# raviraj988/3D-POINT-CLOUD-SEGMENTATION-USING-2D-IMG-SEGMENTATION

Measured on AMD Instinct MI355X. Metric: labelled points/sec (10M pts x 64 views) at 1/2/4/8 GPU; % HBM roofline, higher is better.
Workload: dtype f64; 1 GPU; C3: 10000000 points x 64 ring views, 1024x1024 block64 uint8 masks, nclasses=133, threshold=0.5, filter_classes=None; fused project->sample->vote->segment; points_total=10000000, points_per_gpu=10000000, views=64, xyz_storage=f64, cloud_layout=caller order, cell-sorted inside every step (F3D_FUSE_SORT), exchange=none

## Files before the change

3d-point-cloud-segmentation-using-2d-img-segmentation_amd/csrc/f3d_fuse.hip:

```cpp
#include <hip/hip_runtime.h>
#include <stdint.h>
#include <stdlib.h>
#include <string.h>
#include "f3d.h"
#include "f3d_math.h"
#include "f3d_kernels.h"
#include "f3d_fuse_blocks.h"
#include "f3d_fuse_deal.h"
#include <cstdlib>

#pragma clang fp contract(off)

#define F3D_NO_PREFILL ((int64_t)0x7fffffffffffffffLL)
#define F3D_PART_MAX_GROUPS 16
#ifndef F3D_MID_DENSE
#define F3D_MID_DENSE 8
#endif
#ifndef F3D_NT_CLASSES
#define F3D_NT_CLASSES 1
#endif
#if defined(F3D_EXP_STORE) && F3D_EXP_STORE == 2
#define F3D_STORE_CLASS(p, v) ((void)(v))
#elif defined(F3D_EXP_STORE) && F3D_EXP_STORE == 3
#define F3D_STORE_CLASS(p, v) (reinterpret_cast<uint8_t*>(classes)[(p) - classes] = (uint8_t)(v))
// ... 1357 lines not shown
        if (nclasses + 3 > F3D_BIN32_MAX_CODES) fuse(km2, lds_mid, F3D_BIN32_MAX_CODES + 1, 4 * F3D_PACKED_SMALL_WORDS, one_group ? 4 : 3);
        if (nclasses + 3 > 4 * F3D_PACKED_SMALL_WORDS) fuse(km3, lds_large, 4 * F3D_PACKED_SMALL_WORDS + 1, 4 * F3D_PACKED_LARGE_WORDS, 3);
        if (nclasses + 3 > 4 * F3D_PACKED_LARGE_WORDS) fuse(kf, lds_full, 4 * F3D_PACKED_LARGE_WORDS + 1, 256, 2);
        if (chunk_flags & 2) return hipGetLastError();
        const bool wide = nviews > 255;
        if (wide && !j.masks) return hipErrorInvalidValue;
        auto km = k_fuse_mid<T, V>;
        const size_t lds_tier2 = mid_lds_bytes(words_max);
        if ((e = raise_lds(km, lds_tier2)) != hipSuccess) return e;
        hipLaunchKernelGGL(km, dim3(1024), b, lds_tier2, s, xyz, todo_count, todo, j.views_dev, nviews, j.cmasks, h, w, nclasses, flt.nfilter,
                           flt.cls_dev, j.threshold, j.classes, j.votes, j.err, j.perm, gather, wide ? todo_count + 2 : (unsigned int*)nullptr,
                           wide ? todo2 : (int32_t*)nullptr, todo2_count, j.cb,
                           (const unsigned long long*)umask, (const uint32_t*)park, j.lay.park_slots, j.lay.park_stride);
        if (!wide) return hipGetLastError();
    }
    const unsigned int* exact_count = fast ? todo_count + 2 : todo2_count;
    const int32_t* exact_list = fast ? todo2 : nullptr;
    auto ke = mode == MODE_HIST8 ? k_fuse_exact<T, MODE_HIST8, V> : k_fuse_exact<T, MODE_HIST16, V>;
    if ((e = raise_lds(ke, lds_exact)) != hipSuccess) return e;
    hipLaunchKernelGGL(ke, ge, b, lds_exact, s, xyz, n, exact_count, exact_list, j.views_dev, nviews, j.masks, h, w, nclasses,
                       flt, j.threshold, j.classes, j.votes, j.err, j.perm, gather);
    return hipGetLastError();
}

static f3d_setup_args setup_args_for(const f3d_fuse_job& j, f3d_codebook* cb, bool with_book) {
    const int v0 = j.carry ? j.v0 : 0, cnv = (j.carry ? j.v1 : j.nviews) - v0;
    const fuse_tables tab = fuse_tables_split(j.tables, cnv);
    f3d_setup_args a;
    a.views = j.views_dev + v0; a.nviews = cnv; a.ctabT = tab.ctabT; a.vtabT = tab.vtabT; a.cb = cb; a.threshold = j.threshold;
    a.todo_count = v0 == 0 ? f3d_fuse_todo::counters(j.todo) : (unsigned int*)nullptr;
    a.lut_nclasses = with_book ? j.nclasses : 0;
    a.lut_book = with_book ? pick_book(j.flt, j.votes != nullptr) : -1;
    a.flt = j.flt;
    if (!with_book) { a.flt.nfilter = 0; a.flt.cls_dev = nullptr; a.flt.cls_host = nullptr; for (int k = 0; k < 8; ++k) a.flt.cls[k] = -1; }
    return a;
}

hipError_t f3d_launch_fuse_setup(const f3d_fuse_job& j, f3d_codebook* cb, bool with_book) {
    if ((j.carry ? j.v1 - j.v0 : j.nviews) <= 0) return hipSuccess;
    if (with_book && (j.nclasses < 0 || j.nclasses > F3D_CODE_MAX_NCLASSES)) return hipErrorInvalidValue;
    hipLaunchKernelGGL(k_fuse_setup, dim3(with_book ? 9 : 8), dim3(F3D_BLOCK), 0, j.stream, setup_args_for(j, cb, with_book));
    return hipGetLastError();
}

hipError_t f3d_launch_cell_sort_with_riders(f3d_fuse_job& j, uint8_t* coded, f3d_codebook* cb, int32_t* perm, void* sort_scratch) {
    if (j.nviews <= 0 || j.n <= 0) return hipErrorInvalidValue;
    if (j.nclasses < 0 || j.nclasses > F3D_CODE_MAX_NCLASSES || ((uintptr_t)coded & 7)) return hipErrorInvalidValue;
    f3d_sort_riders r;
    r.masks = j.masks; r.mask_bytes = (int64_t)j.nviews * j.h * j.w; r.cb = cb;
    r.presence = pick_book(j.flt, j.votes != nullptr) == 1;
    const int64_t fill = unlabelled_after_remap(j.nclasses, j.flt);
    j.filled = fill != F3D_NO_PREFILL;
    r.classes = j.filled ? j.classes : nullptr; r.n = j.n; r.fill_value = fill;
    const int pb = r.presence ? f3d_grid_for(r.mask_bytes >> 4, F3D_RIDER_THREADS * F3D_RIDER_UNROLL_1, F3D_RIDER_BLOCKS_1) : 0;
    const int fb = j.filled ? f3d_grid_for(j.n, F3D_RIDER_THREADS * 8, F3D_RIDER_BLOCKS_1) : 0;
    r.pass1_blocks = pb > fb ? pb : fb;
    r.setup = setup_args_for(j, cb, true); r.setup_blocks = 9;
    r.coded = coded; r.V = j.nviews; r.H = j.h; r.W = j.w;
    r.code_blocks = f3d_grid_for((int64_t)j.nviews * (int64_t)(f3d_coded_plane(j.h, j.w) / 8), F3D_RIDER_THREADS * F3D_RIDER_UNROLL, F3D_RIDER_BLOCKS_2);
    return f3d_launch_cell_sort(j.xyz, j.dtype, j.n, nullptr, perm, sort_scratch, j.stream, &r);
}

hipError_t f3d_launch_fuse(const f3d_fuse_job& j) {
    if (j.n <= 0) return hipSuccess;
    const int mode = j.nviews <= 255 ? MODE_HIST8 : MODE_HIST16;
    const int64_t ntiles = (j.n + F3D_BLOCK * 2 - 1) / (F3D_BLOCK * 2);
    int grid = (int)(ntiles < F3D_FUSE_GRID ? ntiles : F3D_FUSE_GRID);
    grid = (grid + 7) & ~7;
    if (j.carry && j.votes) return hipErrorInvalidValue;
    if (j.carry) return j.dtype == F3D_F64 ? launch_fuse_t<double, false, true>(j, mode, grid) : launch_fuse_t<float, false, true>(j, mode, grid);
    if (j.dtype == F3D_F64) return j.votes ? launch_fuse_t<double, true, false>(j, mode, grid) : launch_fuse_t<double, false, false>(j, mode, grid);
    return j.votes ? launch_fuse_t<float, true, false>(j, mode, grid) : launch_fuse_t<float, false, false>(j, mode, grid);
}

hipError_t f3d_launch_fastpath_audit(const void* xyz, int dtype, int64_t n, const f3d_view* views_dev, int nviews, int w, int h,
                                     unsigned long long* stats_dev, hipStream_t s) {
    hipError_t e = hipMemsetAsync(stats_dev, 0, 4 * sizeof(unsigned long long), s);
    if (e != hipSuccess || n <= 0) return e;
    const dim3 g(f3d_grid_for(n, F3D_BLOCK, F3D_GRID_CAP)), b(F3D_BLOCK);
    if (dtype == F3D_F64) hipLaunchKernelGGL(k_fastpath_audit<double>, g, b, 0, s, (const double*)xyz, n, views_dev, nviews, w, h, stats_dev);
    else hipLaunchKernelGGL(k_fastpath_audit<float>, g, b, 0, s, (const float*)xyz, n, views_dev, nviews, w, h, stats_dev);
    return hipGetLastError();
}
```

3d-point-cloud-segmentation-using-2d-img-segmentation_amd/csrc/f3d_fuse_blocks.h:

```cpp
#pragma once
#include <hip/hip_runtime.h>
#include <stdint.h>
#include "f3d.h"
#include "f3d_kernels.h"

#define F3D_RIDER_THREADS 512
#ifndef F3D_RIDER_UNROLL
#define F3D_RIDER_UNROLL 6
#endif
#ifndef F3D_RIDER_UNROLL_1
#define F3D_RIDER_UNROLL_1 8
#endif
#ifndef F3D_RIDER_BLOCKS_1
#define F3D_RIDER_BLOCKS_1 256
#endif
#ifndef F3D_RIDER_BLOCKS_2
#define F3D_RIDER_BLOCKS_2 1024
#endif
#define F3D_CODE_NONE 0u
#define F3D_CODE_BAD 1u
#define F3D_CODE_OTHER 2u
#define F3D_VHEAD 15

__host__ __device__ inline int f3d_coded_pitch(int W) { return ((W + 7) >> 3) + 2; }
__host__ __device__ inline size_t f3d_coded_plane(int H, int W) { return (size_t)(((H + 7) >> 3) + 2) * (size_t)f3d_coded_pitch(W) * 64; }

__device__ __forceinline__ void f3d_presence_publish(const unsigned* blkset, f3d_codebook* __restrict__ cb) {
    if (threadIdx.x < 8) {
        const unsigned want = blkset[threadIdx.x];
        const unsigned have = __hip_atomic_load(&cb->presence[threadIdx.x], __ATOMIC_RELAXED, __HIP_MEMORY_SCOPE_AGENT);
        if (want & ~have) atomicOr(&cb->presence[threadIdx.x], want);
    }
}

template <bool VEC>
__device__ __forceinline__ void f3d_presence_block(const uint8_t* __restrict__ src, int64_t nbytes, f3d_codebook* __restrict__ cb,
                                                   int blk, int nblk, int nthr) {
    unsigned long long m0 = 0, m1 = 0, m2 = 0, m3 = 0;
    auto mark = [&](unsigned l) {
        const unsigned long long bit = 1ull << (l & 63u);
        const unsigned q = l >> 6;
        m0 |= q == 0u ? bit : 0ull; m1 |= q == 1u ? bit : 0ull; m2 |= q == 2u ? bit : 0ull; m3 |= q == 3u ? bit : 0ull;
    };
    const int64_t stride = (int64_t)nblk * nthr;
    if (VEC) {
        const int64_t nw = nbytes >> 3;
        const uint64_t* w = reinterpret_cast<const uint64_t*>(src);
        uint64_t last = ~0ull;
        for (int64_t k = (int64_t)blk * nthr + threadIdx.x; k < nw; k += stride) {
            const uint64_t x = w[k];
            if (x == last) continue;
            if (x == (x & 0xFFull) * 0x0101010101010101ull) { mark((unsigned)(x & 0xFFull)); last = x; continue; }
#pragma unroll
            for (int c = 0; c < 8; ++c) mark((unsigned)(x >> (8 * c)) & 0xFFu);
        }
        if (blk == 0 && (int64_t)threadIdx.x < (nbytes & 7)) mark(src[(nw << 3) + threadIdx.x]);
    } else {
        for (int64_t k = (int64_t)blk * nthr + threadIdx.x; k < nbytes; k += stride) mark(src[k]);
    }
#pragma unroll
    for (int off = 32; off >= 1; off >>= 1) {
        m0 |= __shfl_xor(m0, off, 64); m1 |= __shfl_xor(m1, off, 64); m2 |= __shfl_xor(m2, off, 64); m3 |= __shfl_xor(m3, off, 64);
    }
    __shared__ unsigned blkset[8];
    if (threadIdx.x < 8) blkset[threadIdx.x] = 0u;
    __syncthreads();
    if ((threadIdx.x & 63) == 0) {
        const unsigned long long m[4] = {m0, m1, m2, m3};
#pragma unroll
        for (int q = 0; q < 4; ++q) {
// ... 167 lines not shown
                xs[u] = in[u] ? *reinterpret_cast<const uint64_t*>(rows + ry * W + tx * 8) : 0ull;
            }
#pragma unroll
            for (int u = 0; u < UNROLL; ++u) {
                const int e = e0 + 64 * u;
                if (e >= per_row) break;
                const uint64_t x = xs[u];
                uint64_t o = 0;
                if (in[u]) {
                    if (x == ((x << 8) | (x >> 56))) { const uint32_t c = (uint32_t)lut[x & 0xFFull] * 0x01010101u; o = ((uint64_t)c << 32) | c; }
                    else {
#pragma unroll
                        for (int c = 0; c < 8; ++c) o |= (uint64_t)lut[(x >> (8 * c)) & 0xFFull] << (8 * c);
                    }
                }
                out[e] = o;
            }
        }
    }
}

__device__ __forceinline__ void f3d_fill_labels_block(int64_t* __restrict__ classes, int64_t n, int64_t value, int blk, int nblk, int nthr) {
    for (int64_t i = (int64_t)blk * nthr + threadIdx.x; i < n; i += (int64_t)nblk * nthr)
        __builtin_nontemporal_store(value, &classes[i]);
}

struct f3d_setup_args {
    const f3d_view* views; int nviews;
    float* ctabT; double* vtabT;
    f3d_codebook* cb; double threshold;
    unsigned int* todo_count;
    int lut_nclasses, lut_book;
    f3d_filter_args flt;
};
__device__ __forceinline__ void f3d_fuse_setup_block(const f3d_setup_args& a, int blk, int nblk, int nthr) {
    if (a.lut_book >= 0 && blk == nblk - 1) { f3d_code_lut_block(a.cb, a.lut_nclasses, a.lut_book, a.flt); return; }
    if (blk == 0) {
        f3d_threshold_table(a.cb, a.threshold);
        if (a.todo_count && threadIdx.x < 4) a.todo_count[threadIdx.x] = 0u;
    }
    const int ngroups = (a.nviews + 63) >> 6;
    const int nsetup = a.lut_book >= 0 ? nblk - 1 : nblk;
    for (int k = blk * nthr + threadIdx.x; k < ngroups * 64 * 39; k += nsetup * nthr) {
        const int v = k / 39, f = k - v * 39, g = v >> 6, l = v & 63;
        const f3d_view& vw = a.views[v < a.nviews ? v : a.nviews - 1];
        if (f < 24) a.ctabT[(g * 24 + f) * 64 + l] = reinterpret_cast<const float*>(&vw.cull_n32[0][0])[f];
        else a.vtabT[(g * F3D_VHEAD + (f - 24)) * 64 + l] = reinterpret_cast<const double*>(&vw)[f - 24];
    }
}

struct f3d_sort_riders {
    const uint8_t* masks; int64_t mask_bytes; f3d_codebook* cb; bool presence;
    int64_t* classes; int64_t n; int64_t fill_value; int pass1_blocks;
    f3d_setup_args setup; int setup_blocks;
    uint8_t* coded; int V, H, W; int code_blocks;
};
```

3d-point-cloud-segmentation-using-2d-img-segmentation_amd/csrc/f3d_kernels.h:

```cpp
#pragma once
#include <hip/hip_runtime.h>
#include <float.h>
#include <stdint.h>
#include <atomic>
#include "f3d.h"
#include "f3d_math.h"

#define F3D_DEVERR_FUSE 1
#define F3D_DEVERR_VOTE 2
#define F3D_DEVERR_CC 4
#define F3D_DEVERR_FLOOD 8
#define F3D_DEVERR_COLOR 16
#define F3D_DEVERR_QUADS 32
#define F3D_DEVERR_GROW 64
#define F3D_DEVERR_PVOTE 128
#define F3D_DEVERR_MESH 256
#define F3D_DEVERR_ZVOTE 512
#define F3D_DEVERR_PLANES 1024
#define F3D_DEVERR_RASTER 2048
#define F3D_DEVERR_SMOOTH 4096
#define F3D_DEVERR_LIFT 8192
#define F3D_DEVERR_ALL 16383
#define F3D_PLANES_PER_LAUNCH 16
#define F3D_OBB_MAX_BOXES 4096
// ... 266 lines not shown
hipError_t f3d_launch_inside_polyhedra(const void* xyz, int dtype, int64_t n, const f3d_plane_args& pa, uint8_t* inside,
                                       hipStream_t s);
#define F3D_CODE_MAX_NCLASSES 253
struct f3d_fuse_todo {
    size_t bytes, list2_off, umask_off, park_off;
    int park_slots, park_stride, ngroups;
    static unsigned int* counters(void* base) { return reinterpret_cast<unsigned int*>(base); }
    static int32_t* list(void* base) { return reinterpret_cast<int32_t*>(reinterpret_cast<char*>(base) + 4 * sizeof(unsigned int)); }
    int32_t* list2(void* base) const { return reinterpret_cast<int32_t*>(reinterpret_cast<char*>(base) + list2_off); }
    unsigned long long* umask(void* base) const { return reinterpret_cast<unsigned long long*>(reinterpret_cast<char*>(base) + umask_off); }
    uint32_t* park(void* base) const { return reinterpret_cast<uint32_t*>(reinterpret_cast<char*>(base) + park_off); }
};
f3d_fuse_todo f3d_fuse_todo_layout(int64_t n, int nviews, int nclasses);
size_t f3d_fuse_tables_bytes(int nviews);
size_t f3d_fuse_carry_bytes(int64_t n, int nclasses);
struct f3d_fuse_occupancy {
    struct entry { const void* kernel; size_t lds; int blocks_per_cu; } e[32];
    int n, cus;
};
struct f3d_fuse_job {
    const void* xyz; int dtype; int64_t n; const int32_t* perm; bool gather;
    const f3d_view* views_dev; int nviews, v0, v1;
    const uint8_t *masks, *cmasks; int h, w;
    int nclasses; f3d_filter_args flt; double threshold;
    int64_t* classes; uint16_t* votes; int* err;
    void* todo; f3d_fuse_todo lay;
    const f3d_codebook* cb; void* tables; uint32_t* carry; void* xyz_keep;
    hipStream_t stream;
    bool filled;
    f3d_fuse_occupancy* occ;
};
hipError_t f3d_launch_fuse(const f3d_fuse_job& job);
hipError_t f3d_launch_fuse_setup(const f3d_fuse_job& job, f3d_codebook* cb, bool with_book);
hipError_t f3d_launch_code_masks_with_setup(const f3d_fuse_job& job, uint8_t* coded, f3d_codebook* cb);
hipError_t f3d_launch_mask_presence(const uint8_t* src, int64_t nbytes, f3d_codebook* cb, hipStream_t s);
hipError_t f3d_launch_presence_bytes(f3d_codebook* cb, uint8_t* bytes256, bool to_bytes, hipStream_t s);
hipError_t f3d_launch_code_book(f3d_codebook* cb, int nclasses, const f3d_filter_args& flt, bool want_votes, hipStream_t s);
hipError_t f3d_launch_code_planes(const uint8_t* src, uint8_t* dst, int nviews, int h, int w, const f3d_codebook* cb, hipStream_t s);
size_t f3d_coded_masks_bytes(int nviews, int h, int w);
hipError_t f3d_launch_fastpath_audit(const void* xyz, int dtype, int64_t n, const f3d_view* views_dev, int nviews, int w, int h,
                                     unsigned long long* stats_dev, hipStream_t s);
size_t f3d_sort_scratch_bytes(int64_t n);
struct f3d_sort_riders;
hipError_t f3d_launch_cell_sort(const void* xyz, int dtype, int64_t n, void* sorted_xyz, int32_t* perm, void* scratch, hipStream_t s,
                                const f3d_sort_riders* riders = nullptr);
struct f3d_block_role { bool rider; int index; };
__host__ __device__ inline f3d_block_role f3d_rider_role(unsigned b, unsigned grid, unsigned extra) {
    const unsigned before = (unsigned)(((unsigned long long)b * extra) / grid);
    const unsigned upto = (unsigned)(((unsigned long long)(b + 1) * extra) / grid);
    f3d_block_role r;
    r.rider = upto != before;
    r.index = r.rider ? (int)before : (int)(b - before);
    return r;
}
hipError_t f3d_launch_cell_sort_with_riders(f3d_fuse_job& job, uint8_t* coded, f3d_codebook* cb, int32_t* perm, void* sort_scratch);
hipError_t f3d_launch_components(const int64_t* classes, int64_t n, const int64_t* offs, const int32_t* nbrs, int32_t* parent,
                                 int64_t* root, int* err, hipStream_t s, int errbit = F3D_DEVERR_CC);
size_t f3d_flood_scratch_bytes(int64_t n);
hipError_t f3d_launch_flood_order(const int64_t* classes, int64_t n, const int64_t* offs, const int32_t* nbrs, const int64_t* inst, int k,
                                  int64_t* root, int64_t* order, int64_t* coffs, uint8_t* flags, void* scratch, int* err, int64_t stats[4],
                                  hipStream_t s);
struct f3d_color_args {
    double thr[3];
    int max_level;
    int nneutral;
    int64_t neutral[F3D_COLOR_MAX_NEUTRAL];
};
size_t f3d_color_scratch_bytes(int64_t n);
hipError_t f3d_launch_color_segment(const void* colors, int dtype, int64_t n, const int64_t* offs, const int32_t* nbrs, int64_t* ids,
                                    const int64_t* seeds, int64_t nseeds, const f3d_color_args& a, void* scratch, int64_t* stats_dev, int* err,
                                    hipStream_t s);
struct f3d_grow_args {
    double thr[3];
    double sma0[3];
    int64_t npts0;
    int max_level;
    int seeds_given;
};
#define F3D_GROW_MAX_POINTS (0x7fffffffLL - 2048)
size_t f3d_grow_scratch_bytes(int64_t n);
hipError_t f3d_launch_region_grow(const void* values, int dtype, int nchan, int64_t n, const int64_t* offs, const int32_t* nbrs,
                                  const int64_t* seeds, int64_t nseeds, const f3d_grow_args& a, void* scratch, int64_t* cluster,
                                  int64_t* count_dev, int* err, hipStream_t s);
hipError_t f3d_launch_plane_distance(const double* pts, int64_t n, const double pp[3], const double nr[3], double* out, hipStream_t s);
size_t f3d_graph_bbox_bytes(void);
hipError_t f3d_launch_graph_bbox(const void* xyz, int dtype, int64_t n, void* partial, int* nblocks, hipStream_t s);
int f3d_graph_reduce_bbox(const void* partial_host, int nblocks, double lo[3], double hi[3]);
size_t f3d_graph_scratch_bytes(int64_t n, int64_t ncells);
hipError_t f3d_launch_graph_count(const void* xyz, int dtype, int64_t n, const f3d_gridsearch& gs, void* scratch, int64_t* offsets,
                                  hipStream_t s);
hipError_t f3d_launch_graph_fill(int64_t n, const f3d_gridsearch& gs, const void* scratch, const int64_t* offsets, int32_t* nbrs,
                                 hipStream_t s);
hipError_t f3d_launch_graph_grid(const void* xyz, int dtype, int64_t n, const f3d_graphgrid& g, void* scratch, f3d_gridview* view,
                                 hipStream_t s);
size_t f3d_query_scratch_bytes(int64_t m, int64_t n, int64_t ncells);
hipError_t f3d_launch_query_count(const void* data, int ddtype, int64_t m, const void* queries, int qdtype, int64_t n, const f3d_gridsearch& gs,
                                  void* scratch, int64_t* offsets, int64_t* words_host, hipStream_t s);
hipError_t f3d_launch_query_fill(const void* queries, int qdtype, int64_t m, int64_t n, const f3d_gridsearch& gs, void* scratch,
                                 const int64_t* offsets, int32_t* nbrs, hipStream_t s);
#define F3D_KNN_MAX_K 32
hipError_t f3d_launch_knn_flag(const void* queries, int qdtype, int64_t n, unsigned* flag, hipStream_t s);
hipError_t f3d_launch_knn_query(const void* queries, int qdtype, int64_t n, int k, const f3d_gridview& gv, const f3d_gridsearch& gs,
                                int32_t* idx, double* dist2 , int32_t* counts , hipStream_t s);
hipError_t f3d_launch_knn_labels(const void* queries, int qdtype, int64_t n, int k, const f3d_gridview& gv, const f3d_gridsearch& gs,
                                 const int64_t* labels, int64_t fill, int64_t* out, int32_t* support , hipStream_t s);

// ... 225 lines not shown
```

3d-point-cloud-segmentation-using-2d-img-segmentation_amd/csrc/f3d_sort.hip:

```cpp
#include <hip/hip_runtime.h>
#include <stdint.h>
#include <cstring>
#include "f3d.h"
#include "f3d_kernels.h"
#include "f3d_fuse_blocks.h"

namespace {

constexpr int SB = 256;
#define F3D_SORT_KEY_BITS 16
typedef uint16_t sort_key_t;

struct bbox6 { double lo[3], hi[3]; };

template <typename T>
__global__ __launch_bounds__(SB) void k_bbox_partial(const T* __restrict__ xyz, int64_t n, int64_t stride, bbox6* __restrict__ partial) {
    double lo[3] = {1e300, 1e300, 1e300}, hi[3] = {-1e300, -1e300, -1e300};
#pragma unroll 4
    for (int64_t i = ((int64_t)blockIdx.x * SB + threadIdx.x) * stride; i < n; i += (int64_t)gridDim.x * SB * stride) {
#pragma unroll
        for (int c = 0; c < 3; ++c) {
            const double x = (double)xyz[3 * i + c];
            if (fabs(x) < 1e300) { lo[c] = fmin(lo[c], x); hi[c] = fmax(hi[c], x); }
        }
// ... 113 lines not shown
#define F3D_RK_THREADS 256
#endif
constexpr int RK_SMALL_THREADS = 512;
template <typename T, int RK_THREADS>
__global__ __launch_bounds__(RK_THREADS) void k_rs_keys(const T* __restrict__ xyz, int64_t n, const bbox6* __restrict__ partial, int nparts,
                                                         sort_key_t* __restrict__ keys, uint32_t* __restrict__ blkhist, int ntiles) {
    __shared__ uint32_t hist[256];
    __shared__ f3d_cellgrid sg;
    __shared__ uint16_t lut[3][RS_LUT];
    constexpr int RK_ROUNDS = RS_TILE / RK_THREADS;
    static_assert(RK_THREADS >= 64 && RK_THREADS * RK_ROUNDS == RS_TILE, "the key kernel's block must cover a tile");
    const int wave = threadIdx.x >> 6, lane = threadIdx.x & 63;
    if (wave == 0) grid_from_partials(partial, nparts, &sg);
    for (int d = threadIdx.x; d < 256; d += RK_THREADS) hist[d] = 0u;
    __syncthreads();
    f3d_cellgrid g = sg;
#pragma unroll
    for (int c = 0; c < 3; ++c) {
        g.dim[c] = __builtin_amdgcn_readfirstlane(g.dim[c]);
        g.bits[c] = __builtin_amdgcn_readfirstlane(g.bits[c]);
    }
    const bool tables = g.dim[0] <= RS_LUT && g.dim[1] <= RS_LUT && g.dim[2] <= RS_LUT;
    if (tables) {
        for (int c = 0; c < 3; ++c)
            for (int i = threadIdx.x; i < g.dim[c]; i += RK_THREADS) lut[c][i] = (uint16_t)spread_axis((uint32_t)i, c, g.bits);
        __syncthreads();
    }
    const float lo[3] = {(float)g.lo[0], (float)g.lo[1], (float)g.lo[2]};
    const float inv[3] = {(float)g.inv_cell[0], (float)g.inv_cell[1], (float)g.inv_cell[2]};
#pragma unroll 8
    for (int r = 0; r < RK_ROUNDS; ++r) {
        const int64_t i = (int64_t)blockIdx.x * RS_TILE + (int64_t)wave * (RK_ROUNDS * 64) + r * 64 + lane;
        if (i < n) {
            uint32_t key;
            if (tables) {
                int idx[3]; bool ok;
                cell_index(xyz + 3 * i, lo, inv, g.dim, idx, ok);
                key = ok ? ((uint32_t)lut[0][idx[0]] | lut[1][idx[1]] | lut[2][idx[2]]) : ((1u << F3D_SORT_KEY_BITS) - 1u);
            } else {
                key = cell_of(xyz + 3 * i, g);
            }
            keys[i] = (sort_key_t)key;
            atomicAdd(&hist[key & 0xFFu], 1u);
        }
    }
    __syncthreads();
    for (int d = threadIdx.x; d < 256; d += RK_THREADS) blkhist[(size_t)d * ntiles + blockIdx.x] = hist[d];
}

template <typename R> struct rs_rec;
template <> struct rs_rec<uint32_t> { static constexpr int shift = 24; static constexpr uint32_t imask = 0xFFFFFFu; };
template <> struct rs_rec<uint64_t> { static constexpr int shift = 32; static constexpr uint64_t imask = 0xFFFFFFFFull; };

template <typename R>
__global__ __launch_bounds__(RS_THREADS) void k_rs_hist2(const R* __restrict__ recs, int64_t n, uint32_t* __restrict__ blkhist, int ntiles) {
    __shared__ uint32_t hist[256];
    const int wave = threadIdx.x >> 6, lane = threadIdx.x & 63;
    if (threadIdx.x < 256) hist[threadIdx.x] = 0u;
    __syncthreads();
#pragma unroll 4
    for (int r = 0; r < RS_ROUNDS; ++r) {
        const int64_t i = rs_item(blockIdx.x, wave, r, lane);
        if (i < n) atomicAdd(&hist[(uint32_t)(recs[i] >> rs_rec<R>::shift) & 0xFFu], 1u);
    }
    __syncthreads();
    if (threadIdx.x < 256) blkhist[(size_t)threadIdx.x * ntiles + blockIdx.x] = hist[threadIdx.x];
}

__device__ __forceinline__ void rs_scan_row(uint32_t* __restrict__ blkhist, int ntiles, uint32_t* __restrict__ tot, int d) {
    __shared__ uint32_t part[256];
    uint32_t* row = blkhist + (size_t)d * ntiles;
    const int per = (ntiles + 255) / 256;
    const int lo = threadIdx.x * per, hi = min(ntiles, lo + per);
    uint32_t sum = 0;
    for (int k = lo; k < hi; ++k) sum += row[k];
    part[threadIdx.x] = sum;
    __syncthreads();
    for (int off = 1; off < 256; off <<= 1) {
        const uint32_t v = threadIdx.x >= off ? part[threadIdx.x - off] : 0u;
        __syncthreads();
        part[threadIdx.x] += v;
        __syncthreads();
    }
    uint32_t run = part[threadIdx.x] - sum;
    for (int k = lo; k < hi; ++k) { const uint32_t c = row[k]; row[k] = run; run += c; }
    if (threadIdx.x == 255) tot[d] = part[255];
}
__global__ __launch_bounds__(256) void k_rs_scan(uint32_t* __restrict__ blkhist, int ntiles, uint32_t* __restrict__ tot) {
    rs_scan_row(blkhist, ntiles, tot, blockIdx.x);
}

__global__ __launch_bounds__(256) void k_rs_scan_setup(uint32_t* __restrict__ blkhist, int ntiles, uint32_t* __restrict__ tot, f3d_setup_args setup, int extra) {
    const f3d_block_role role = f3d_rider_role(blockIdx.x, gridDim.x, (unsigned)extra);
    if (role.rider) { f3d_fuse_setup_block(setup, role.index, extra, 256); return; }
    rs_scan_row(blkhist, ntiles, tot, role.index);
}

__device__ __forceinline__ uint32_t rs_excl_scan256(uint32_t v, uint32_t* wsum ) {
    const int lane = threadIdx.x & 63, wave = threadIdx.x >> 6;
    uint32_t inc = v;
#pragma unroll
    for (int off = 1; off < 64; off <<= 1) { const uint32_t o = __shfl_up(inc, off, 64); if (lane >= off) inc += o; }
    __syncthreads();
    if (lane == 63 && wave < 4) wsum[wave] = inc;
    __syncthreads();
    uint32_t before = 0u;
    for (int w = 0; w < 4; ++w) before += (w < wave) ? wsum[w] : 0u;
    return before + inc - v;
}

__device__ __forceinline__ void rs_round_order() {
    __builtin_amdgcn_fence(__ATOMIC_ACQ_REL, "workgroup", "local");
    __builtin_amdgcn_wave_barrier();
}

template <int PASS, typename R>
__device__ __forceinline__ void rs_scatter_tile(const sort_key_t* __restrict__ keys, const R* __restrict__ recs_in, int64_t n,
                                                const uint32_t* __restrict__ offs, const uint32_t* __restrict__ tot, int ntiles,
                                                R* __restrict__ recs_out, uint32_t* __restrict__ perm_out, const int tile) {
    __shared__ uint32_t wcount[RS_WAVES][256];
    __shared__ uint32_t gdelta[256];
    __shared__ uint32_t wsum[4];
    extern __shared__ unsigned long long rs_dyn[];
    R* srec = reinterpret_cast<R*>(rs_dyn);
    uint8_t* sdig = reinterpret_cast<uint8_t*>(srec + RS_TILE);
    static_assert((size_t)RS_WAVES * 256 * sizeof(unsigned long long) <= (size_t)RS_TILE * sizeof(uint32_t), "the lane masks must fit under the records");
    static_assert(RS_TILE <= (1 << 16), "a tile position is packed into 16 bits of dig[r]");
    const int wave = threadIdx.x >> 6, lane = threadIdx.x & 63;
    unsigned long long* const wmask = rs_dyn + wave * 256;
    const int d_own = threadIdx.x & 255;
    const bool own = threadIdx.x < 256;
    const uint32_t t_d = own ? tot[d_own] : 0u;
    const uint32_t o_d = own ? offs[(size_t)d_own * ntiles + tile] : 0u;
    for (int k = threadIdx.x; k < RS_WAVES * 256; k += RS_THREADS) { (&wcount[0][0])[k] = 0u; rs_dyn[k] = 0ull; }
    __syncthreads();
    uint32_t dig[RS_ROUNDS];
    R val[RS_ROUNDS];
#pragma unroll
    for (int r = 0; r < RS_ROUNDS; ++r) {
        const int64_t i = rs_item(tile, wave, r, lane);
        dig[r] = 0xFFFFFFFFu; val[r] = 0;
        if (i < n) {
            if (PASS == 1) { const uint32_t k = keys[i]; dig[r] = k & 0xFFu; val[r] = ((R)(k >> 8) << rs_rec<R>::shift) | (R)i; }
            else { val[r] = recs_in[i]; dig[r] = (uint32_t)(val[r] >> rs_rec<R>::shift) & 0xFFu; }
            atomicAdd(&wcount[wave][dig[r]], 1u);
        }
    }
    __syncthreads();
    {
        uint32_t c_d = 0u;
        if (own) for (int w = 0; w < RS_WAVES; ++w) c_d += wcount[w][d_own];
        const uint32_t gstart = rs_excl_scan256(t_d, wsum);
        const uint32_t lstart = rs_excl_scan256(c_d, wsum);
        if (own) {
            gdelta[d_own] = gstart + o_d - lstart;
            uint32_t run = lstart;
            for (int w = 0; w < RS_WAVES; ++w) { const uint32_t c = wcount[w][d_own]; wcount[w][d_own] = run; run += c; }
        }
    }
    __syncthreads();
    const unsigned long long below = (1ull << lane) - 1ull;
#pragma unroll
    for (int r = 0; r < RS_ROUNDS; ++r) {
        const uint32_t d = dig[r];
        const bool live = d != 0xFFFFFFFFu;
        if (live) __hip_atomic_fetch_or(&wmask[d], 1ull << lane, __ATOMIC_RELAXED, __HIP_MEMORY_SCOPE_WORKGROUP);
        rs_round_order();
        unsigned long long m = 0ull;
        uint32_t base = 0u;
        if (live) {
            m = __hip_atomic_load(&wmask[d], __ATOMIC_RELAXED, __HIP_MEMORY_SCOPE_WORKGROUP);
            base = __hip_atomic_load(&wcount[wave][d], __ATOMIC_RELAXED, __HIP_MEMORY_SCOPE_WORKGROUP);
        }
        rs_round_order();
        const uint32_t rank = (uint32_t)__popcll(m & below);
        if (live && rank == 0u) {
            __hip_atomic_store(&wcount[wave][d], base + (uint32_t)__popcll(m), __ATOMIC_RELAXED, __HIP_MEMORY_SCOPE_WORKGROUP);
            __hip_atomic_store(&wmask[d], 0ull, __ATOMIC_RELAXED, __HIP_MEMORY_SCOPE_WORKGROUP);
        }
        rs_round_order();
        if (live) dig[r] = (d << 16) | (base + rank);
    }
    __syncthreads();
#pragma unroll
    for (int r = 0; r < RS_ROUNDS; ++r) {
        if (dig[r] != 0xFFFFFFFFu) {
            const uint32_t pos = dig[r] & 0xFFFFu;
            srec[pos] = val[r];
            if (PASS == 1) sdig[pos] = (uint8_t)(dig[r] >> 16);
        }
    }
    __syncthreads();
    const int64_t left = n - (int64_t)tile * RS_TILE;
    const int count = (int)(left < RS_TILE ? left : RS_TILE);
#pragma unroll 4
    for (int j = threadIdx.x; j < count; j += RS_THREADS) {
        const R rec = srec[j];
        if (PASS == 1) recs_out[(uint32_t)j + gdelta[sdig[j]]] = rec;
        else perm_out[(uint32_t)j + gdelta[(uint32_t)(rec >> rs_rec<R>::shift) & 0xFFu]] = (uint32_t)(rec & rs_rec<R>::imask);
    }
}

template <int PASS, typename R>
__global__ __launch_bounds__(RS_THREADS) void k_rs_scatter(const sort_key_t* __restrict__ keys, const R* __restrict__ recs_in, int64_t n,
                                                            const uint32_t* __restrict__ offs, const uint32_t* __restrict__ tot, int ntiles,
                                                            R* __restrict__ recs_out, uint32_t* __restrict__ perm_out) {
    rs_scatter_tile<PASS, R>(keys, recs_in, n, offs, tot, ntiles, recs_out, perm_out, blockIdx.x);
}

template <int PASS, typename R>
__global__ __launch_bounds__(RS_THREADS) void k_rs_scatter_ride(const sort_key_t* __restrict__ keys, const R* __restrict__ recs_in, int64_t n,
                                                                 const uint32_t* __restrict__ offs, const uint32_t* __restrict__ tot, int ntiles,
                                                                 R* __restrict__ recs_out, uint32_t* __restrict__ perm_out,
                                                                 const uint8_t* __restrict__ masks, int64_t mask_bytes, f3d_codebook* __restrict__ cb,
                                                                 uint8_t* __restrict__ coded, int V, int H, int W,
                                                                 int64_t* __restrict__ classes, int64_t nfill, int64_t fill_value, int extra) {
    const f3d_block_role role = f3d_rider_role(blockIdx.x, gridDim.x, (unsigned)extra);
    if (role.rider) {
        if (PASS == 1) {
            if (masks) {
                if (!((uintptr_t)masks & 7)) f3d_presence_block_wide<F3D_RIDER_UNROLL_1>(masks, mask_bytes, cb, role.index, extra, RS_THREADS);
                else f3d_presence_block<false>(masks, mask_bytes, cb, role.index, extra, RS_THREADS);
            }
            if (classes) f3d_fill_labels_block(classes, nfill, fill_value, role.index, extra, RS_THREADS);
        } else {
            if (!(W & 7) && !((uintptr_t)masks & 7)) f3d_code_masks_block_rows<F3D_RIDER_UNROLL>(masks, coded, V, H, W, cb, role.index, extra, RS_THREADS);
            else f3d_code_masks_block<false>(masks, coded, V, H, W, cb, role.index, extra, RS_THREADS);
        }
        return;
    }
    rs_scatter_tile<PASS, R>(keys, recs_in, n, offs, tot, ntiles, recs_out, perm_out, role.index);
}

template <typename T>
__global__ __launch_bounds__(SB) void k_gather_xyz(const T* __restrict__ xyz, int64_t n, const int32_t* __restrict__ perm,
                                                    T* __restrict__ sorted) {
    for (int64_t i = (int64_t)blockIdx.x * SB + threadIdx.x; i < n; i += (int64_t)gridDim.x * SB) {
        const size_t src = (size_t)perm[i];
        sorted[3 * i] = xyz[3 * src]; sorted[3 * i + 1] = xyz[3 * src + 1]; sorted[3 * i + 2] = xyz[3 * src + 2];
    }
}

struct sort_layout {
    size_t partial, keys, recs, hist, tot, total;
    int ntiles;
    bool wide;
};

sort_layout layout_for(int64_t n) {
    sort_layout L;
    f3d_carve c;
    L.ntiles = (int)((n + RS_TILE - 1) / RS_TILE);
    L.wide = n > (1 << 24);
    L.partial = c.take(64 * sizeof(bbox6));
    L.keys = c.take((size_t)n * sizeof(sort_key_t));
    L.recs = c.take((size_t)n * (L.wide ? 8 : 4));
    L.hist = c.take((size_t)256 * L.ntiles * 4);
    L.tot = c.take(256 * 4);
    L.total = c.off;
    return L;
}

template <typename R>
hipError_t run_passes(const sort_layout& L, char* base, int64_t n, int32_t* perm, hipStream_t s, const f3d_sort_riders* rd) {
    const sort_key_t* keys = reinterpret_cast<const sort_key_t*>(base + L.keys);
    R* recs = reinterpret_cast<R*>(base + L.recs);
    uint32_t* hist = reinterpret_cast<uint32_t*>(base + L.hist);
    uint32_t* tot = reinterpret_cast<uint32_t*>(base + L.tot);
    const dim3 gt(L.ntiles), bt(RS_THREADS);
    const size_t lds1 = (size_t)RS_TILE * sizeof(R) + RS_TILE, lds2 = (size_t)RS_TILE * sizeof(R);
    if (lds1 > 48 * 1024) {
        hipError_t e = hipFuncSetAttribute((const void*)k_rs_scatter<1, R>, hipFuncAttributeMaxDynamicSharedMemorySize, (int)lds1);
        if (e == hipSuccess) e = hipFuncSetAttribute((const void*)k_rs_scatter<2, R>, hipFuncAttributeMaxDynamicSharedMemorySize, (int)lds2);
        if (e != hipSuccess) return e;
    }
    if (rd) {
        if (lds1 > 48 * 1024) {
            hipError_t e = hipFuncSetAttribute((const void*)k_rs_scatter_ride<1, R>, hipFuncAttributeMaxDynamicSharedMemorySize, (int)lds1);
            if (e == hipSuccess) e = hipFuncSetAttribute((const void*)k_rs_scatter_ride<2, R>, hipFuncAttributeMaxDynamicSharedMemorySize, (int)lds2);
            if (e != hipSuccess) return e;
        }
        hipLaunchKernelGGL(k_rs_scan, dim3(256), dim3(256), 0, s, hist, L.ntiles, tot);
        if (rd->pass1_blocks > 0)
            hipLaunchKernelGGL((k_rs_scatter_ride<1, R>), dim3(L.ntiles + rd->pass1_blocks), bt, lds1, s, keys, (const R*)nullptr, n, hist, tot, L.ntiles, recs,
                               (uint32_t*)nullptr, rd->presence ? rd->masks : (const uint8_t*)nullptr, rd->mask_bytes, rd->cb, (uint8_t*)nullptr, 0, 0, 0,
                               rd->classes, rd->n, rd->fill_value, rd->pass1_blocks);
        else hipLaunchKernelGGL((k_rs_scatter<1, R>), gt, bt, lds1, s, keys, (const R*)nullptr, n, hist, tot, L.ntiles, recs, (uint32_t*)nullptr);
        hipLaunchKernelGGL(k_rs_hist2<R>, gt, bt, 0, s, recs, n, hist, L.ntiles);
        hipLaunchKernelGGL(k_rs_scan_setup, dim3(256 + rd->setup_blocks), dim3(256), 0, s, hist, L.ntiles, tot, rd->setup, rd->setup_blocks);
        hipLaunchKernelGGL((k_rs_scatter_ride<2, R>), dim3(L.ntiles + rd->code_blocks), bt, lds2, s, (const sort_key_t*)nullptr, recs, n, hist, tot, L.ntiles,
                           (R*)nullptr, reinterpret_cast<uint32_t*>(perm), rd->masks, rd->mask_bytes, rd->cb, rd->coded, rd->V, rd->H, rd->W,
                           (int64_t*)nullptr, (int64_t)0, (int64_t)0, rd->code_blocks);
        return hipGetLastError();
    }
    hipLaunchKernelGGL(k_rs_scan, dim3(256), dim3(256), 0, s, hist, L.ntiles, tot);
    hipLaunchKernelGGL((k_rs_scatter<1, R>), gt, bt, lds1, s, keys, (const R*)nullptr, n, hist, tot, L.ntiles, recs, (uint32_t*)nullptr);
    hipLaunchKernelGGL(k_rs_hist2<R>, gt, bt, 0, s, recs, n, hist, L.ntiles);
    hipLaunchKernelGGL(k_rs_scan, dim3(256), dim3(256), 0, s, hist, L.ntiles, tot);
    hipLaunchKernelGGL((k_rs_scatter<2, R>), gt, bt, lds2, s, (const sort_key_t*)nullptr, recs, n, hist, tot, L.ntiles, (R*)nullptr, reinterpret_cast<uint32_t*>(perm));
    return hipGetLastError();
}

}

size_t f3d_sort_scratch_bytes(int64_t n) { return layout_for(n < 1 ? 1 : n).total; }

hipError_t f3d_launch_cell_sort(const void* xyz, int dtype, int64_t n, void* sorted_xyz, int32_t* perm, void* scratch, hipStream_t s,
                                const f3d_sort_riders* riders) {
    if (n <= 0) return hipSuccess;
    if (n > 0x7fffffffLL) return hipErrorInvalidValue;
    const sort_layout L = layout_for(n);
    char* base = reinterpret_cast<char*>(scratch);
    bbox6* partial = reinterpret_cast<bbox6*>(base + L.partial);
    sort_key_t* keys = reinterpret_cast<sort_key_t*>(base + L.keys);
    uint32_t* hist = reinterpret_cast<uint32_t*>(base + L.hist);
    const int64_t stride = n > (1 << 16) ? n >> 16 : 1;
    const int64_t sb = ((n + stride - 1) / stride + SB - 1) / SB;
    const int nparts = (int)(sb < 64 ? sb : 64);
    const int gstream = f3d_grid_for(n, SB, 8192);
    const dim3 gt(L.ntiles);
    const bool small = L.ntiles < 512;
    if (dtype == F3D_F64) {
        hipLaunchKernelGGL(k_bbox_partial<double>, dim3(nparts), dim3(SB), 0, s, (const double*)xyz, n, stride, partial);
        if (small) hipLaunchKernelGGL((k_rs_keys<double, RK_SMALL_THREADS>), gt, dim3(RK_SMALL_THREADS), 0, s, (const double*)xyz, n, partial, nparts, keys, hist, L.ntiles);
        else hipLaunchKernelGGL((k_rs_keys<double, F3D_RK_THREADS>), gt, dim3(F3D_RK_THREADS), 0, s, (const double*)xyz, n, partial, nparts, keys, hist, L.ntiles);
    } else {
        hipLaunchKernelGGL(k_bbox_partial<float>, dim3(nparts), dim3(SB), 0, s, (const float*)xyz, n, stride, partial);
        if (small) hipLaunchKernelGGL((k_rs_keys<float, RK_SMALL_THREADS>), gt, dim3(RK_SMALL_THREADS), 0, s, (const float*)xyz, n, partial, nparts, keys, hist, L.ntiles);
        else hipLaunchKernelGGL((k_rs_keys<float, F3D_RK_THREADS>), gt, dim3(F3D_RK_THREADS), 0, s, (const float*)xyz, n, partial, nparts, keys, hist, L.ntiles);
    }
    hipError_t e = L.wide ? run_passes<uint64_t>(L, base, n, perm, s, riders) : run_passes<uint32_t>(L, base, n, perm, s, riders);
    if (e != hipSuccess) return e;
    if (sorted_xyz) {
        if (dtype == F3D_F64) hipLaunchKernelGGL(k_gather_xyz<double>, dim3(gstream), dim3(SB), 0, s, (const double*)xyz, n, perm, (double*)sorted_xyz);
        else hipLaunchKernelGGL(k_gather_xyz<float>, dim3(gstream), dim3(SB), 0, s, (const float*)xyz, n, perm, (float*)sorted_xyz);
    }
    return hipGetLastError();
}
```

Before: 11.68 billion points/s.

## Rework radix sort passes: vectorized histogram, packed counters, run-based digit lookup, fill rider

Moves the class-label prefill rider out of sort pass 1 and into the histogram kernel for large clouds, and uses a smaller pass-1 rider cap for small inputs. The histogram kernel now loads each tile with 16-byte vector loads. Per-wave digit counters in the scatter are packed as uint16, and the per-element digit byte array is replaced with a run bitmap plus prefix table, so each record's global offset is found with a popcount. Min-waves launch bounds are also added. These aim to cut LDS traffic, pass-1 load imbalance and histogram load cost, at the price of more complex indexing and tighter register limits.

```diff
diff --git a/3d-point-cloud-segmentation-using-2d-img-segmentation_amd/csrc/f3d_fuse.hip b/3d-point-cloud-segmentation-using-2d-img-segmentation_amd/csrc/f3d_fuse.hip
--- a/3d-point-cloud-segmentation-using-2d-img-segmentation_amd/csrc/f3d_fuse.hip
+++ b/3d-point-cloud-segmentation-using-2d-img-segmentation_amd/csrc/f3d_fuse.hip
@@ -1433,8 +1433,11 @@
     const int64_t fill = unlabelled_after_remap(j.nclasses, j.flt);
     j.filled = fill != F3D_NO_PREFILL;
     r.classes = j.filled ? j.classes : nullptr; r.n = j.n; r.fill_value = fill;
-    const int pb = r.presence ? f3d_grid_for(r.mask_bytes >> 4, F3D_RIDER_THREADS * F3D_RIDER_UNROLL_1, F3D_RIDER_BLOCKS_1) : 0;
-    const int fb = j.filled ? f3d_grid_for(j.n, F3D_RIDER_THREADS * 8, F3D_RIDER_BLOCKS_1) : 0;
+    const bool small = j.n < F3D_RIDER_SMALL_POINTS;
+    const int cap1 = small ? F3D_RIDER_BLOCKS_1_SMALL : F3D_RIDER_BLOCKS_1;
+    const int pb = r.presence ? f3d_grid_for(r.mask_bytes >> 4, F3D_RIDER_THREADS * F3D_RIDER_UNROLL_1, cap1) : 0;
+    r.fill_blocks = (j.filled && !small && F3D_RIDER_BLOCKS_FILL > 0) ? f3d_grid_for(j.n, F3D_RIDER_THREADS * 8, F3D_RIDER_BLOCKS_FILL) : 0;
+    const int fb = (j.filled && r.fill_blocks == 0) ? f3d_grid_for(j.n, F3D_RIDER_THREADS * 8, cap1) : 0;
     r.pass1_blocks = pb > fb ? pb : fb;
     r.setup = setup_args_for(j, cb, true); r.setup_blocks = 9;
     r.coded = coded; r.V = j.nviews; r.H = j.h; r.W = j.w;
diff --git a/3d-point-cloud-segmentation-using-2d-img-segmentation_amd/csrc/f3d_fuse_blocks.h b/3d-point-cloud-segmentation-using-2d-img-segmentation_amd/csrc/f3d_fuse_blocks.h
--- a/3d-point-cloud-segmentation-using-2d-img-segmentation_amd/csrc/f3d_fuse_blocks.h
+++ b/3d-point-cloud-segmentation-using-2d-img-segmentation_amd/csrc/f3d_fuse_blocks.h
@@ -16,6 +16,15 @@
 #endif
 #ifndef F3D_RIDER_BLOCKS_2
 #define F3D_RIDER_BLOCKS_2 1024
+#endif
+#ifndef F3D_RIDER_BLOCKS_FILL
+#define F3D_RIDER_BLOCKS_FILL 512
+#endif
+#ifndef F3D_RIDER_SMALL_POINTS
+#define F3D_RIDER_SMALL_POINTS (512 * 8192)
+#endif
+#ifndef F3D_RIDER_BLOCKS_1_SMALL
+#define F3D_RIDER_BLOCKS_1_SMALL 128
 #endif
 #define F3D_CODE_NONE 0u
 #define F3D_CODE_BAD 1u
@@ -289,6 +298,7 @@
 struct f3d_sort_riders {
     const uint8_t* masks; int64_t mask_bytes; f3d_codebook* cb; bool presence;
     int64_t* classes; int64_t n; int64_t fill_value; int pass1_blocks;
+    int fill_blocks;
     f3d_setup_args setup; int setup_blocks;
     uint8_t* coded; int V, H, W; int code_blocks;
 };
diff --git a/3d-point-cloud-segmentation-using-2d-img-segmentation_amd/csrc/f3d_kernels.h b/3d-point-cloud-segmentation-using-2d-img-segmentation_amd/csrc/f3d_kernels.h
--- a/3d-point-cloud-segmentation-using-2d-img-segmentation_amd/csrc/f3d_kernels.h
+++ b/3d-point-cloud-segmentation-using-2d-img-segmentation_amd/csrc/f3d_kernels.h
@@ -342,6 +342,18 @@
     r.rider = upto != before;
     r.index = r.rider ? (int)before : (int)(b - before);
     return r;
+}
+struct f3d_run_span { unsigned word, bit, first, last; };
+__host__ __device__ inline f3d_run_span f3d_run_span_of(unsigned start, unsigned count, unsigned nwords) {
+    f3d_run_span s;
+    s.word = start >> 6; s.bit = start & 63u;
+    s.first = (start >> 6) + 1u;
+    s.last = (start + count) >> 6;
+    if (s.last > nwords - 1u) s.last = nwords - 1u;
+    return s;
+}
+__host__ __device__ inline unsigned f3d_run_at(unsigned long long word, unsigned before, unsigned bit) {
+    return before + (unsigned)__builtin_popcountll(word & ((2ull << bit) - 1ull)) - 1u;
 }
 hipError_t f3d_launch_cell_sort_with_riders(f3d_fuse_job& job, uint8_t* coded, f3d_codebook* cb, int32_t* perm, void* sort_scratch);
 hipError_t f3d_launch_components(const int64_t* classes, int64_t n, const int64_t* offs, const int32_t* nbrs, int32_t* parent,
diff --git a/3d-point-cloud-segmentation-using-2d-img-segmentation_amd/csrc/f3d_sort.hip b/3d-point-cloud-segmentation-using-2d-img-segmentation_amd/csrc/f3d_sort.hip
--- a/3d-point-cloud-segmentation-using-2d-img-segmentation_amd/csrc/f3d_sort.hip
+++ b/3d-point-cloud-segmentation-using-2d-img-segmentation_amd/csrc/f3d_sort.hip
@@ -189,19 +189,38 @@
 template <> struct rs_rec<uint32_t> { static constexpr int shift = 24; static constexpr uint32_t imask = 0xFFFFFFu; };
 template <> struct rs_rec<uint64_t> { static constexpr int shift = 32; static constexpr uint64_t imask = 0xFFFFFFFFull; };
 
+#ifndef F3D_RH_THREADS
+#define F3D_RH_THREADS 512
+#endif
+constexpr int RH_THREADS = F3D_RH_THREADS;
 template <typename R>
-__global__ __launch_bounds__(RS_THREADS) void k_rs_hist2(const R* __restrict__ recs, int64_t n, uint32_t* __restrict__ blkhist, int ntiles) {
+__global__ __launch_bounds__(RH_THREADS) void k_rs_hist2(const R* __restrict__ recs, int64_t n, uint32_t* __restrict__ blkhist, int ntiles,
+                                                          int64_t* __restrict__ classes, int64_t nfill, int64_t fill_value, int extra) {
+    const f3d_block_role role = f3d_rider_role(blockIdx.x, gridDim.x, (unsigned)extra);
+    if (role.rider) { f3d_fill_labels_block(classes, nfill, fill_value, role.index, extra, RH_THREADS); return; }
     __shared__ uint32_t hist[256];
-    const int wave = threadIdx.x >> 6, lane = threadIdx.x & 63;
+    constexpr int PER = 16 / sizeof(R);
+    constexpr int LOADS = RS_TILE / (RH_THREADS * PER);
+    static_assert(RH_THREADS >= 256 && LOADS * RH_THREADS * PER == RS_TILE, "the histogram kernel's block must cover a tile");
+    typedef R vec_t __attribute__((ext_vector_type(PER)));
     if (threadIdx.x < 256) hist[threadIdx.x] = 0u;
     __syncthreads();
-#pragma unroll 4
-    for (int r = 0; r < RS_ROUNDS; ++r) {
-        const int64_t i = rs_item(blockIdx.x, wave, r, lane);
-        if (i < n) atomicAdd(&hist[(uint32_t)(recs[i] >> rs_rec<R>::shift) & 0xFFu], 1u);
-    }
-    __syncthreads();
-    if (threadIdx.x < 256) blkhist[(size_t)threadIdx.x * ntiles + blockIdx.x] = hist[threadIdx.x];
+    const int64_t base = (int64_t)role.index * RS_TILE;
+    if (base + RS_TILE <= n && !((uintptr_t)recs & 15)) {
+        const vec_t* __restrict__ src = reinterpret_cast<const vec_t*>(recs + base);
+        vec_t v[LOADS];
+#pragma unroll
+        for (int r = 0; r < LOADS; ++r) v[r] = src[r * RH_THREADS + threadIdx.x];
+#pragma unroll
+        for (int r = 0; r < LOADS; ++r)
+#pragma unroll
+            for (int c = 0; c < PER; ++c) atomicAdd(&hist[(uint32_t)(v[r][c] >> rs_rec<R>::shift) & 0xFFu], 1u);
+    } else {
+        const int64_t end = base + RS_TILE < n ? base + RS_TILE : n;
+        for (int64_t i = base + threadIdx.x; i < end; i += RH_THREADS) atomicAdd(&hist[(uint32_t)(recs[i] >> rs_rec<R>::shift) & 0xFFu], 1u);
+    }
+    __syncthreads();
+    if (threadIdx.x < 256) blkhist[(size_t)threadIdx.x * ntiles + role.index] = hist[threadIdx.x];
 }
 
 __device__ __forceinline__ void rs_scan_row(uint32_t* __restrict__ blkhist, int ntiles, uint32_t* __restrict__ tot, int d) {
@@ -251,25 +270,33 @@
     __builtin_amdgcn_wave_barrier();
 }
 
+constexpr int RS_WORDS = RS_TILE / 64;
+template <int PASS, typename R> constexpr size_t rs_dyn_lds() { return (size_t)RS_TILE * sizeof(R) + (PASS == 1 ? RS_WORDS * (sizeof(unsigned long long) + sizeof(uint16_t)) : 0); }
+template <typename R> constexpr int rs_min_waves() { return sizeof(R) == 4 ? 8 : 2; }
+
 template <int PASS, typename R>
 __device__ __forceinline__ void rs_scatter_tile(const sort_key_t* __restrict__ keys, const R* __restrict__ recs_in, int64_t n,
                                                 const uint32_t* __restrict__ offs, const uint32_t* __restrict__ tot, int ntiles,
                                                 R* __restrict__ recs_out, uint32_t* __restrict__ perm_out, const int tile) {
-    __shared__ uint32_t wcount[RS_WAVES][256];
+    __shared__ uint16_t wcount[RS_WAVES][256];
     __shared__ uint32_t gdelta[256];
     __shared__ uint32_t wsum[4];
     extern __shared__ unsigned long long rs_dyn[];
     R* srec = reinterpret_cast<R*>(rs_dyn);
-    uint8_t* sdig = reinterpret_cast<uint8_t*>(srec + RS_TILE);
+    unsigned long long* starts = reinterpret_cast<unsigned long long*>(srec + RS_TILE);
+    uint16_t* before = reinterpret_cast<uint16_t*>(starts + RS_WORDS);
     static_assert((size_t)RS_WAVES * 256 * sizeof(unsigned long long) <= (size_t)RS_TILE * sizeof(uint32_t), "the lane masks must fit under the records");
-    static_assert(RS_TILE <= (1 << 16), "a tile position is packed into 16 bits of dig[r]");
+    static_assert(RS_TILE <= (1 << 16) - 1 && RS_ROUNDS * 64 < (1 << 16), "a tile position and a wave's count fit 16 bits");
     const int wave = threadIdx.x >> 6, lane = threadIdx.x & 63;
     unsigned long long* const wmask = rs_dyn + wave * 256;
     const int d_own = threadIdx.x & 255;
     const bool own = threadIdx.x < 256;
     const uint32_t t_d = own ? tot[d_own] : 0u;
     const uint32_t o_d = own ? offs[(size_t)d_own * ntiles + tile] : 0u;
-    for (int k = threadIdx.x; k < RS_WAVES * 256; k += RS_THREADS) { (&wcount[0][0])[k] = 0u; rs_dyn[k] = 0ull; }
+    typedef uint32_t __attribute__((may_alias)) pair_t;
+    pair_t* const wpair = reinterpret_cast<pair_t*>(&wcount[0][0]);
+    for (int k = threadIdx.x; k < RS_WAVES * 256; k += RS_THREADS) { if (k < RS_WAVES * 128) wpair[k] = 0u; rs_dyn[k] = 0ull; }
+    if (PASS == 1 && threadIdx.x < RS_WORDS) { starts[threadIdx.x] = 0ull; if (threadIdx.x == 0) before[0] = 0; }
     __syncthreads();
     uint32_t dig[RS_ROUNDS];
     R val[RS_ROUNDS];
@@ -280,7 +307,7 @@
         if (i < n) {
             if (PASS == 1) { const uint32_t k = keys[i]; dig[r] = k & 0xFFu; val[r] = ((R)(k >> 8) << rs_rec<R>::shift) | (R)i; }
             else { val[r] = recs_in[i]; dig[r] = (uint32_t)(val[r] >> rs_rec<R>::shift) & 0xFFu; }
-            atomicAdd(&wcount[wave][dig[r]], 1u);
+            atomicAdd(&wpair[wave * 128 + (dig[r] >> 1)], 1u << (16 * (dig[r] & 1u)));
         }
     }
     __syncthreads();
@@ -288,11 +315,21 @@
         uint32_t c_d = 0u;
         if (own) for (int w = 0; w < RS_WAVES; ++w) c_d += wcount[w][d_own];
         const uint32_t gstart = rs_excl_scan256(t_d, wsum);
-        const uint32_t lstart = rs_excl_scan256(c_d, wsum);
+        const uint32_t both = rs_excl_scan256(PASS == 1 ? (c_d | (c_d ? 1u << 16 : 0u)) : c_d, wsum);
+        const uint32_t lstart = both & 0xFFFFu;
         if (own) {
-            gdelta[d_own] = gstart + o_d - lstart;
+            const uint32_t gd = gstart + o_d - lstart;
+            if (PASS == 1) {
+                if (c_d) {
+                    const uint32_t rank = both >> 16;
+                    const f3d_run_span sp = f3d_run_span_of(lstart, c_d, RS_WORDS);
+                    __hip_atomic_fetch_or(&starts[sp.word], 1ull << sp.bit, __ATOMIC_RELAXED, __HIP_MEMORY_SCOPE_WORKGROUP);
+                    gdelta[rank] = gd;
+                    for (uint32_t w = sp.first; w <= sp.last; ++w) before[w] = (uint16_t)(rank + 1u);
+                }
+            } else gdelta[d_own] = gd;
             uint32_t run = lstart;
-            for (int w = 0; w < RS_WAVES; ++w) { const uint32_t c = wcount[w][d_own]; wcount[w][d_own] = run; run += c; }
+            for (int w = 0; w < RS_WAVES; ++w) { const uint32_t c = wcount[w][d_own]; wcount[w][d_own] = (uint16_t)run; run += c; }
         }
     }
     __syncthreads();
@@ -312,7 +349,7 @@
         rs_round_order();
         const uint32_t rank = (uint32_t)__popcll(m & below);
         if (live && rank == 0u) {
-            __hip_atomic_store(&wcount[wave][d], base + (uint32_t)__popcll(m), __ATOMIC_RELAXED, __HIP_MEMORY_SCOPE_WORKGROUP);
+            __hip_atomic_store(&wcount[wave][d], (uint16_t)(base + (uint32_t)__popcll(m)), __ATOMIC_RELAXED, __HIP_MEMORY_SCOPE_WORKGROUP);
             __hip_atomic_store(&wmask[d], 0ull, __ATOMIC_RELAXED, __HIP_MEMORY_SCOPE_WORKGROUP);
         }
         rs_round_order();
@@ -320,33 +357,28 @@
     }
     __syncthreads();
 #pragma unroll
-    for (int r = 0; r < RS_ROUNDS; ++r) {
-        if (dig[r] != 0xFFFFFFFFu) {
-            const uint32_t pos = dig[r] & 0xFFFFu;
-            srec[pos] = val[r];
-            if (PASS == 1) sdig[pos] = (uint8_t)(dig[r] >> 16);
-        }
-    }
+    for (int r = 0; r < RS_ROUNDS; ++r)
+        if (dig[r] != 0xFFFFFFFFu) srec[dig[r] & 0xFFFFu] = val[r];
     __syncthreads();
     const int64_t left = n - (int64_t)tile * RS_TILE;
     const int count = (int)(left < RS_TILE ? left : RS_TILE);
 #pragma unroll 4
     for (int j = threadIdx.x; j < count; j += RS_THREADS) {
         const R rec = srec[j];
-        if (PASS == 1) recs_out[(uint32_t)j + gdelta[sdig[j]]] = rec;
+        if (PASS == 1) recs_out[(uint32_t)j + gdelta[f3d_run_at(starts[j >> 6], before[j >> 6], (unsigned)j & 63u)]] = rec;
         else perm_out[(uint32_t)j + gdelta[(uint32_t)(rec >> rs_rec<R>::shift) & 0xFFu]] = (uint32_t)(rec & rs_rec<R>::imask);
     }
 }
 
 template <int PASS, typename R>
-__global__ __launch_bounds__(RS_THREADS) void k_rs_scatter(const sort_key_t* __restrict__ keys, const R* __restrict__ recs_in, int64_t n,
+__global__ __launch_bounds__(RS_THREADS, rs_min_waves<R>()) void k_rs_scatter(const sort_key_t* __restrict__ keys, const R* __restrict__ recs_in, int64_t n,
                                                             const uint32_t* __restrict__ offs, const uint32_t* __restrict__ tot, int ntiles,
                                                             R* __restrict__ recs_out, uint32_t* __restrict__ perm_out) {
     rs_scatter_tile<PASS, R>(keys, recs_in, n, offs, tot, ntiles, recs_out, perm_out, blockIdx.x);
 }
 
 template <int PASS, typename R>
-__global__ __launch_bounds__(RS_THREADS) void k_rs_scatter_ride(const sort_key_t* __restrict__ keys, const R* __restrict__ recs_in, int64_t n,
+__global__ __launch_bounds__(RS_THREADS, rs_min_waves<R>()) void k_rs_scatter_ride(const sort_key_t* __restrict__ keys, const R* __restrict__ recs_in, int64_t n,
                                                                  const uint32_t* __restrict__ offs, const uint32_t* __restrict__ tot, int ntiles,
                                                                  R* __restrict__ recs_out, uint32_t* __restrict__ perm_out,
                                                                  const uint8_t* __restrict__ masks, int64_t mask_bytes, f3d_codebook* __restrict__ cb,
@@ -405,7 +437,7 @@
     uint32_t* hist = reinterpret_cast<uint32_t*>(base + L.hist);
     uint32_t* tot = reinterpret_cast<uint32_t*>(base + L.tot);
     const dim3 gt(L.ntiles), bt(RS_THREADS);
-    const size_t lds1 = (size_t)RS_TILE * sizeof(R) + RS_TILE, lds2 = (size_t)RS_TILE * sizeof(R);
+    const size_t lds1 = rs_dyn_lds<1, R>(), lds2 = rs_dyn_lds<2, R>();
     if (lds1 > 48 * 1024) {
         hipError_t e = hipFuncSetAttribute((const void*)k_rs_scatter<1, R>, hipFuncAttributeMaxDynamicSharedMemorySize, (int)lds1);
         if (e == hipSuccess) e = hipFuncSetAttribute((const void*)k_rs_scatter<2, R>, hipFuncAttributeMaxDynamicSharedMemorySize, (int)lds2);
@@ -418,12 +450,14 @@
             if (e != hipSuccess) return e;
         }
         hipLaunchKernelGGL(k_rs_scan, dim3(256), dim3(256), 0, s, hist, L.ntiles, tot);
+        const bool fill2 = rd->classes && rd->fill_blocks > 0;
         if (rd->pass1_blocks > 0)
             hipLaunchKernelGGL((k_rs_scatter_ride<1, R>), dim3(L.ntiles + rd->pass1_blocks), bt, lds1, s, keys, (const R*)nullptr, n, hist, tot, L.ntiles, recs,
                                (uint32_t*)nullptr, rd->presence ? rd->masks : (const uint8_t*)nullptr, rd->mask_bytes, rd->cb, (uint8_t*)nullptr, 0, 0, 0,
-                               rd->classes, rd->n, rd->fill_value, rd->pass1_blocks);
+                               fill2 ? (int64_t*)nullptr : rd->classes, rd->n, rd->fill_value, rd->pass1_blocks);
         else hipLaunchKernelGGL((k_rs_scatter<1, R>), gt, bt, lds1, s, keys, (const R*)nullptr, n, hist, tot, L.ntiles, recs, (uint32_t*)nullptr);
-        hipLaunchKernelGGL(k_rs_hist2<R>, gt, bt, 0, s, recs, n, hist, L.ntiles);
+        const int fb = fill2 ? rd->fill_blocks : 0;
+        hipLaunchKernelGGL(k_rs_hist2<R>, dim3(L.ntiles + fb), dim3(RH_THREADS), 0, s, recs, n, hist, L.ntiles, fill2 ? rd->classes : (int64_t*)nullptr, rd->n, rd->fill_value, fb);
         hipLaunchKernelGGL(k_rs_scan_setup, dim3(256 + rd->setup_blocks), dim3(256), 0, s, hist, L.ntiles, tot, rd->setup, rd->setup_blocks);
         hipLaunchKernelGGL((k_rs_scatter_ride<2, R>), dim3(L.ntiles + rd->code_blocks), bt, lds2, s, (const sort_key_t*)nullptr, recs, n, hist, tot, L.ntiles,
                            (R*)nullptr, reinterpret_cast<uint32_t*>(perm), rd->masks, rd->mask_bytes, rd->cb, rd->coded, rd->V, rd->H, rd->W,
@@ -432,7 +466,7 @@
     }
     hipLaunchKernelGGL(k_rs_scan, dim3(256), dim3(256), 0, s, hist, L.ntiles, tot);
     hipLaunchKernelGGL((k_rs_scatter<1, R>), gt, bt, lds1, s, keys, (const R*)nullptr, n, hist, tot, L.ntiles, recs, (uint32_t*)nullptr);
-    hipLaunchKernelGGL(k_rs_hist2<R>, gt, bt, 0, s, recs, n, hist, L.ntiles);
+    hipLaunchKernelGGL(k_rs_hist2<R>, gt, dim3(RH_THREADS), 0, s, recs, n, hist, L.ntiles, (int64_t*)nullptr, (int64_t)0, (int64_t)0, 0);
     hipLaunchKernelGGL(k_rs_scan, dim3(256), dim3(256), 0, s, hist, L.ntiles, tot);
     hipLaunchKernelGGL((k_rs_scatter<2, R>), gt, bt, lds2, s, (const sort_key_t*)nullptr, recs, n, hist, tot, L.ntiles, (R*)nullptr, reinterpret_cast<uint32_t*>(perm));
     return hipGetLastError();
```

Result: faster. 11.86 billion points/s (median of 6 runs) (+1.5%).
